# ywq/psnerf

Measured on AMD Instinct MI355X. Metric: ray-samples/sec (train step) on BEAR stage2, higher is better.
Workload: dtype f32

## Files before the change

include/psnerf_hip.h:

```cpp
#ifndef PSNERF_HIP_H
#define PSNERF_HIP_H

#include <stdint.h>

#ifdef __cplusplus
extern "C" {
#endif

#define PSN_OK 0
#define PSN_E_ARG (-1)
#define PSN_E_LAUNCH (-2)
#define PSN_E_UNSUPPORTED (-3)

const char* psn_last_error(void);
int psn_version(void);

int psn_composite_fwd(const float* alpha, const float* rgb, int64_t n_rays, int n_samples, int white_bg,
                      float* weights, float* rgb_out, float* acc_out, void* stream);
int psn_composite_bwd(const float* alpha, const float* rgb, const float* d_rgb_out, const float* d_acc_out,
                      int64_t n_rays, int n_samples, int white_bg, float* d_alpha, float* d_rgb, void* stream);

int psn_pe_encode(const float* x, int64_t n, int n_freqs, float scale, float* out, int out_stride, void* stream);
int psn_app_input(const float* p, const float* v, const float* normal, int64_t n, int n_freqs, float* out, void* stream);

// ... 135 lines not shown
    int n_layers;
    int n_out;
    int out_act;
    int in_kt_a;
    int in_kt_b;
    int init_stride;
    int w_format;
    PsnMlpLayer layers[PSN_MLP_MAX_LAYERS];
} PsnMlpDesc;

int psn_mlp_pack_layer(const float* W, int64_t ldw, int rows, int cols, int transpose, int n_mt, int k_tiles, float* dst,
                       void* stream);

#define PSN_PACK_MAX_ITEMS 24
typedef struct {
    const float* W;
    float* dst;
    int64_t ldw;
    int rows, cols, transpose, n_mt, k_tiles;
    int format;
} PsnPackItem;
int psn_mlp_pack_layers(int n_items, const PsnPackItem* items, void* stream);

typedef struct {
    const float* tab_a; int64_t a_div, a_mod; const float* tab_b; int64_t b_div, b_mod; const float* init_a; const float* init_b;
    float* const* save_ptrs; unsigned long long* const* save_bits_ptrs; int64_t save_row0;
    const float* const* mask_ptrs; const float* const* aux2_ptrs; float* const* save2_ptrs;
    const float* act_init; int64_t act_init_rows; const float* rk_coef; const float* rk_basis; int rk_k; const uint32_t* dump_tiles;
    int64_t n_rows; float* out; const float* live_count; int64_t live_period;
} PsnMlpLaunch;
typedef struct { int chain, width16, src, trim, from_a, x3, tb_lds, pm_groups; int64_t blocks, pm_period; } PsnMlpPath;
int psn_mlp_launch(const PsnMlpDesc* desc, const float* packed_w, const float* packed_b, const PsnMlpLaunch* launch, PsnMlpPath* path,
                   void* stream);
int psn_mlp_last_path(PsnMlpPath* path);
int psn_mlp_block_order(int point_major);

#define PSN_SCATTER_MAX_ITEMS 16
typedef struct {
    const float* rows;
    float* dense;
    int64_t row_stride, col_stride;
    int B, C;
    float fill;
} PsnScatterItem;
int psn_scatter_rows(int n_items, const PsnScatterItem* items, const int* inv, int64_t N, int64_t Ns, void* stream);
int psn_gather_rows(int n_items, const PsnScatterItem* items, const int64_t* idx, int64_t N, int64_t Ns, void* stream);
int psn_gather_rows_valid(int n_items, const PsnScatterItem* items, const int64_t* idx, const int* inv, int64_t N, int64_t Ns, void* stream);

int psn_secant_step(const float* occ, float tau, float* d_pred, float* d_low, float* d_high, float* f_low, float* f_high,
                    const float* origin, const float* dir, float* p_mid, int64_t n, void* stream);

int psn_first_crossing(const float* occ, const float* far, const float* u, const float* omu, float near, float tau,
// ... 272 lines not shown
```

psnerf_amd/csrc/mlp_infer.hip:

```cpp
#include "common.h"
#include <stdlib.h>
#include <atomic>

namespace psn {

struct InferArgs {
    PsnMlpDesc d;
    const float* w;
    const float* b;
    const float* ta;
    int64_t a_div, a_mod;
    const float* tb;
    int64_t b_div, b_mod;
    const float* init_a;
    const float* init_b;
    int64_t n_rows;
    float* out;
    int n_bias;
    float* save[PSN_MLP_MAX_LAYERS];
    int64_t save_row0;
    const float* mask[PSN_MLP_MAX_LAYERS];
    const float* aux2[PSN_MLP_MAX_LAYERS];
    float* save2[PSN_MLP_MAX_LAYERS];
    const float* act_init;
// ... 2 lines not shown
    const float* rk_coef;
    const float* rk_basis;
    int rk_k;
    const long long* n_rows_dev;
    const int64_t* out_rows;
    const float* ray_o;
    const float* ray_d;
    const float* bracket;
    float tau, pe_scale;
    int n_iter, pe_octaves;
    const float* far;
    const float* u;
    const float* omu;
    float near;
    int n_steps;
    int* skip;
    unsigned long long* n_blocks;
    const float* live_count;
    int64_t live_period;
    unsigned long long* save_bits[PSN_MLP_MAX_LAYERS];
    int tb_lds;
    int64_t pm_period;
    int pm_groups;
};

constexpr int kStageFloats = 8192;
constexpr int kWaves = 4;

template <int NMT, int NACC, bool ASMDMA, typename RequestNext>
__device__ __forceinline__ void stage_compute(floatx4 (&acc)[NACC], const floatx4& b0, const floatx4& b1,
                                              const float4* __restrict__ wl, int lane, RequestNext request_next) {
    if constexpr (NMT >= 8) {
        constexpr int GE = NMT / 8;
        constexpr int NG = 2 * GE;
        float4 a[2][8];
#pragma unroll
        for (int m = 0; m < 8; ++m) a[0][m] = wl[m * 64 + lane];
        __builtin_amdgcn_sched_barrier(0);
        constexpr int NPW = NMT / 2;
        if constexpr (ASMDMA) {
#pragma unroll
            for (int g = 0; g < NG; ++g) {
                const int e = g / GE, m0 = (g % GE) * 8;
                const floatx4& bs = e ? b1 : b0;
                const float4(&ag)[8] = a[g & 1];
#pragma unroll
// ... 171 lines not shown
    } else {
    const unsigned voff = lane * 16;
    switch (j & 3) {
        case 0: lds_dma_16<0>(base, lds, voff); break;
        case 1: lds_dma_16<1024>(base, lds, voff); break;
        case 2: lds_dma_16<2048>(base, lds, voff); break;
        default: lds_dma_16<3072>(base, lds, voff); break;
    }
    }
}
template <int NBLK, bool ASMDMA>
__device__ __forceinline__ void stage_load(const float* __restrict__ gsrc, float* lds_dst, int wave, int lane) {
#pragma unroll
    for (int j = 0; j < NBLK / kWaves; ++j) stage_piece<NBLK, ASMDMA>(gsrc, lds_dst, wave, lane, j);
}

__device__ __forceinline__ floatx4 ld4(const float* p) {
    float4 t = *reinterpret_cast<const float4*>(p);
    floatx4 v;
    v[0] = t.x; v[1] = t.y; v[2] = t.z; v[3] = t.w;
    return v;
}
__device__ __forceinline__ void st4(float* p, const floatx4& v) { *reinterpret_cast<float4*>(p) = make_float4(v[0], v[1], v[2], v[3]); }

template <int CODE, int NMT, bool FROMA = false>
__device__ __forceinline__ void chain_activation(floatx4 (&acc)[NMT], floatx4 (&act)[NMT], const float* __restrict__ p1,
                                                 const float* __restrict__ p2, float* __restrict__ d1, float* __restrict__ d2,
                                                 const uint32_t m1, const uint32_t m2, const unsigned long long sign_bits = 0) {
    constexpr bool kFromA = FROMA && (CODE == PSN_ACT_MUL_AUX || CODE == PSN_ACT_MUL2 || CODE == PSN_ACT_SOFTPLUS_BWD);
    constexpr bool kNeed1 = CODE == PSN_ACT_RELU_MASK || CODE == PSN_ACT_MUL_AUX || CODE == PSN_ACT_MUL2 || CODE == PSN_ACT_SOFTPLUS_BWD;
    constexpr bool kNeed2 = CODE == PSN_ACT_MUL2 || CODE == PSN_ACT_SOFTPLUS_BWD;
    constexpr bool kSecond = CODE == PSN_ACT_SOFTPLUS100 || CODE == PSN_ACT_MUL2 || CODE == PSN_ACT_MUL_AUX;
    floatx4 t1[NMT], t2[NMT];
    if constexpr (kNeed1) {
#pragma unroll
        for (int mt = 0; mt < NMT; ++mt) t1[mt] = ld4(p1 + mt * 16);
    }
    if constexpr (kNeed2) {
#pragma unroll
        for (int mt = 0; mt < NMT; ++mt) t2[mt] = ld4(p2 + mt * 16);
    }
    if constexpr (CODE == PSN_ACT_HEAD) {
        if (d1 != nullptr) {
#pragma unroll
            for (int mt = 0; mt < NMT; ++mt)
                if ((m1 >> mt) & 1) st4(d1 + mt * 16, acc[mt]);
// ... 205 lines not shown
    for (int i = tid; i < g.n_bias; i += kWaves * 64) bias_lds[i] = g.b[i];
    const float* tb_lds = nullptr;
    if constexpr (!CHAIN && SRC == 0) {
        if (g.init_b != nullptr && g.tb_lds != 0 && g.n_bias + g.d.init_stride <= PSN_MLP_MAX_LAYERS * 256) {
            const int64_t r_first = blk_ * (kWaves * 16), r_last_ = r_first + kWaves * 16 - 1;
            const int64_t r_last = r_last_ < n_rows_eff ? r_last_ : n_rows_eff - 1;
            if (r_first / g.b_div == r_last / g.b_div) {
                const int64_t ib0 = (r_first / g.b_div) % g.b_mod;
                float* dst = bias_lds + PSN_MLP_MAX_LAYERS * 256 - g.d.init_stride;
                const float* src = g.init_b + ib0 * (int64_t)g.d.init_stride;
                for (int i = tid; i < g.d.init_stride; i += kWaves * 64) dst[i] = src[i];
                tb_lds = dst;
            }
        }
    }

    floatx4 act[NMT];
    floatx4 acc[NMT];
#pragma unroll
    for (int mt = 0; mt < NMT; ++mt)
#pragma unroll
        for (int r = 0; r < 4; ++r) act[mt][r] = 0.f;
    if constexpr (CHAIN) {
        if (g.act_init != nullptr) {
            const bool has_row = rowc < g.act_init_rows;
            const float* ap = g.act_init + (has_row ? rowc : 0) * W + 4 * lg;
#pragma unroll
            for (int mt = 0; mt < NMT; ++mt) {
                float4 t = *reinterpret_cast<const float4*>(ap + mt * 16);
                act[mt][0] = has_row ? t.x : 0.f; act[mt][1] = has_row ? t.y : 0.f; act[mt][2] = has_row ? t.z : 0.f; act[mt][3] = has_row ? t.w : 0.f;
            }
#pragma unroll
            for (int mt = 0; mt < NMT; ++mt) asm volatile("" : "+v"(act[mt]));
        }
    }

    int gstage = 0;
    int pending_dump = 0;
    int pending_stages = 0;
    const bool dump_row = row < n_rows_eff && row >= g.save_row0;
    const bool wave_dumps = __builtin_amdgcn_ballot_w64(dump_row) != 0;

#define PSN_STAGE(NMT, B0, B1, S_IDX)                                                                       \
    {                                                                                                       \
         \
        wait_for_weights<NMT>(pending_stages > 0 ? pending_dump : 0);                                       \
// ... 69 lines not shown
                    }
                }
                if (tb_lds != nullptr) {
#pragma unroll
                    for (int mt = 0; mt < NMT; ++mt) {
                        const float4 u = *reinterpret_cast<const float4*>(tb_lds + L.init_off + mt * 16 + 4 * lg);
                        acc[mt][0] += u.x;
                        acc[mt][1] += u.y;
                        acc[mt][2] += u.z;
                        acc[mt][3] += u.w;
                    }
                } else if (init_b_row != nullptr) {
#pragma unroll
                    for (int mt = 0; mt < NMT; ++mt) {
                        float4 u = *reinterpret_cast<const float4*>(init_b_row + L.init_off + mt * 16 + 4 * lg);
                        acc[mt][0] += u.x;
                        acc[mt][1] += u.y;
                        acc[mt][2] += u.z;
                        acc[mt][3] += u.w;
                    }
                }
                if constexpr (CHAIN) {
                    if (g.rk_coef != nullptr) {
                        for (int c = 0; c < g.rk_k; ++c) {
                            const float cf = g.rk_coef[rowc * g.rk_k + c];
                            const float* bp2 = g.rk_basis + (int64_t)c * g.d.init_stride + L.init_off + 4 * lg;
#pragma unroll
                            for (int mt = 0; mt < NMT; ++mt) {
                                const float4 u = *reinterpret_cast<const float4*>(bp2 + mt * 16);
                                acc[mt][0] = fmaf(cf, u.x, acc[mt][0]);
                                acc[mt][1] = fmaf(cf, u.y, acc[mt][1]);
                                acc[mt][2] = fmaf(cf, u.z, acc[mt][2]);
                                acc[mt][3] = fmaf(cf, u.w, acc[mt][3]);
                            }
                        }
                    }
                }
            }
        }
        if (L.n_kt_act > 0) {
#pragma unroll
            for (int kt = 0; kt < NMT / 2 - 1; ++kt) PSN_STAGE(NMT, act[2 * kt], act[2 * kt + 1], kt)
            if (!TRIM || L.n_kt_act == NMT / 2) PSN_STAGE(NMT, act[NMT - 2], act[NMT - 1], NMT / 2 - 1)
        }
        if constexpr (SRC != 0) {
            if (L.n_kt_in > 0) {
                if constexpr (SRC == 2 || SRC == 3) {
                    PSN_STAGE(NMT, xq[0], xq[1], L.n_kt_act)
                    PSN_STAGE(NMT, xq[2], xq[3], L.n_kt_act + 1)
                } else {
#pragma unroll
                    for (int kt = 0; kt < 2; ++kt) {
                        const floatx4 x0 = compute_xin_tile(2 * kt), x1 = compute_xin_tile(2 * kt + 1);
                        PSN_STAGE(NMT, x0, x1, L.n_kt_act + kt)
                    }
                }
            }
        } else if (L.n_kt_in > 0) {
// ... 490 lines not shown
static psn::InferArgs base_args(const PsnMlpDesc& d, const float* packed_w, const float* packed_b, int64_t n_rows, float* out) {
    psn::InferArgs a = {};
    a.d = d; a.w = packed_w; a.b = packed_b; a.a_div = 1; a.a_mod = 1; a.b_div = 1; a.b_mod = 1; a.n_rows = n_rows; a.out = out;
    const int width = d.layers[0].n_mt * 32;
    a.n_bias = d.n_out > 0 ? (d.n_layers - 1) * width + (d.n_out > 32 ? 64 : 32) : d.n_layers * width;
    for (int l = 0; l < PSN_MLP_MAX_LAYERS; ++l) { a.save_tiles[l] = 0xFFFFFFFFu; a.save2_tiles[l] = 0xFFFFFFFFu; }
    return a;
}

static int mlp_infer_plan(const PsnMlpDesc* desc, const float* packed_w, const float* packed_b, const PsnMlpLaunch& o, psn::InferArgs& a,
                          PsnMlpPath& p) {
    using namespace psn;
    p = {};
    PSN_CHECK_ARG(desc && packed_w && packed_b && (o.out || desc->n_out == 0), "mlp_infer: null pointer");
    const PsnMlpDesc& d = *desc;
    PSN_CHECK_ARG(d.n_layers >= 1 && d.n_layers <= PSN_MLP_MAX_LAYERS, "mlp_infer: n_layers=%d", d.n_layers);
    PSN_CHECK_ARG(d.in_kt_a >= 0 && d.in_kt_b >= 0 && d.in_kt_a + d.in_kt_b <= 4, "mlp_infer: input tiles %d+%d", d.in_kt_a, d.in_kt_b);
    bool uses_in = false, uses_init = false;
    for (int l = 0; l < d.n_layers; ++l) {
        uses_in = uses_in || d.layers[l].n_kt_in > 0;
        uses_init = uses_init || d.layers[l].init_off >= 0;
    }
    PSN_CHECK_ARG(!uses_in || (o.tab_a && d.in_kt_a >= 1 && (d.in_kt_b == 0 || o.tab_b)), "mlp_infer: input table missing");
    PSN_CHECK_ARG((o.rk_coef == nullptr) == (o.rk_basis == nullptr) && (o.rk_coef == nullptr ? o.rk_k == 0 : (o.rk_k >= 1 && o.rk_k <= 4)),
                  "mlp_infer: rank-k init needs coefficients, basis and 1 <= k <= 4 (k=%d)", o.rk_k);
    PSN_CHECK_ARG(!uses_init || ((o.init_a || o.rk_coef) && d.init_stride >= 64 && d.init_stride % 4 == 0), "mlp_infer: init table missing");
    PSN_CHECK_ARG((((uintptr_t)o.rk_basis) & 15) == 0, "mlp_infer: rk_basis must be 16-byte aligned");
    PSN_CHECK_ARG((((uintptr_t)o.init_a | (uintptr_t)o.init_b) & 15) == 0, "mlp_infer: init tables must be 16-byte aligned");
    PSN_CHECK_ARG(d.n_out >= 0 && d.n_out <= 64, "mlp_infer: n_out=%d", d.n_out);
    PSN_CHECK_ARG(o.a_div >= 1 && o.a_mod >= 1 && (d.in_kt_b == 0 || (o.b_div >= 1 && o.b_mod >= 1)), "mlp_infer: bad index map");
    PSN_CHECK_ARG((((uintptr_t)o.tab_a | (uintptr_t)o.tab_b | (uintptr_t)packed_w | (uintptr_t)packed_b) & 15) == 0,
                  "mlp_infer: buffers must be 16-byte aligned");
    PSN_CHECK_ARG(o.save_bits_ptrs == nullptr || o.save_ptrs != nullptr, "mlp_infer: save_bits_ptrs needs save_ptrs (the sign bits are those of the dumps)");
    PSN_CHECK_ARG((o.live_count != nullptr) == (o.live_period != 0), "mlp_infer: live_count and live_period go together (live_count %s, period=%lld)",
                  o.live_count ? "given" : "is null", (long long)o.live_period);
    PSN_CHECK_ARG(d.n_out == 0 || d.n_layers >= 2, "mlp_infer: a final layer needs at least one hidden layer in front of it (n_layers=%d)", d.n_layers);
    const int hid = d.layers[0].n_mt;
    PSN_CHECK_ARG(hid == 8 || hid == 4 || hid == 2, "mlp_infer: hidden layers must be 256, 128 or 64 wide (n_mt = 8, 4, 2), got n_mt=%d", hid);
    const int width = hid * 32;
    for (int l = 0; l < d.n_layers; ++l) {
        const PsnMlpLayer& L = d.layers[l];
        const bool last = d.n_out > 0 && l == d.n_layers - 1;
        PSN_CHECK_ARG(L.n_mt == (last ? (d.n_out > 32 ? 2 : 1) : hid), "mlp_infer: layer %d n_mt=%d (hidden layers share one width; final: 1, or 2 for 33..64 outputs)", l, L.n_mt);
        PSN_CHECK_ARG(L.n_kt_in >= 0 && L.n_kt_in <= d.in_kt_a + d.in_kt_b, "mlp_infer: layer %d n_kt_in=%d", l, L.n_kt_in);
        PSN_CHECK_ARG(!last || (L.n_kt_in == 0 && L.n_kt_act == hid), "mlp_infer: the final layer reads the hidden activations only");
        PSN_CHECK_ARG(L.b_off == (int64_t)l * width, "mlp_infer: biases must be packed back to back (one hidden width per layer)");
        PSN_CHECK_ARG(L.n_kt_act == 0 || L.n_kt_act == hid || (L.n_kt_act == hid - 1 && hid > 1), "mlp_infer: layer %d n_kt_act=%d (0, n_mt - 1 or n_mt)", l, L.n_kt_act);
        PSN_CHECK_ARG(l > 0 || L.n_kt_act == 0 || o.act_init != nullptr, "mlp_infer: layer 0 cannot read activations without act_init");
        PSN_CHECK_ARG(L.n_kt_in + L.n_kt_act >= 1 || (l == 0 && L.init_off >= 0 && d.n_layers > 1), "mlp_infer: layer %d has no input", l);
        PSN_CHECK_ARG(L.init_off < 0 || (!last && L.init_off + width <= d.init_stride && L.init_off % 4 == 0), "mlp_infer: layer %d bad init_off", l);
// ... 13 lines not shown
        a.aux2[l] = (o.aux2_ptrs != nullptr && in_range) ? o.aux2_ptrs[l] : nullptr;
        a.save2[l] = (o.save2_ptrs != nullptr && in_range) ? o.save2_ptrs[l] : nullptr;
        PSN_CHECK_ARG(((((uintptr_t)a.mask[l]) | ((uintptr_t)a.aux2[l]) | ((uintptr_t)a.save2[l])) & 15) == 0,
                      "mlp_infer: aux / dump tensors must be 16-byte aligned");
        if (in_range) {
            const int act = d.layers[l].act;
            const bool need1 = act == PSN_ACT_RELU_MASK || act == PSN_ACT_MUL_AUX || act == PSN_ACT_MUL2 || act == PSN_ACT_SOFTPLUS_BWD || act == PSN_ACT_RELU_BITS ||
                               act == PSN_ACT_MUL_AUX_A || act == PSN_ACT_MUL2_A || act == PSN_ACT_SOFTPLUS_BWD_A;
            const bool need2 = act == PSN_ACT_MUL2 || act == PSN_ACT_SOFTPLUS_BWD || act == PSN_ACT_MUL2_A || act == PSN_ACT_SOFTPLUS_BWD_A;
            PSN_CHECK_ARG(act >= PSN_ACT_NONE && act <= PSN_ACT_SOFTPLUS_BWD_A, "mlp_infer: layer %d unknown activation %d", l, act);
            PSN_CHECK_ARG(!need1 || a.mask[l] != nullptr, "mlp_infer: layer %d needs aux operand 1", l);
            PSN_CHECK_ARG(!need2 || a.aux2[l] != nullptr, "mlp_infer: layer %d needs aux operand 2", l);
            PSN_CHECK_ARG(act != PSN_ACT_HEAD || a.save[l] != nullptr, "mlp_infer: a HEAD layer needs a dump tensor");
            const bool second = act == PSN_ACT_SOFTPLUS100 || act == PSN_ACT_MUL_AUX || act == PSN_ACT_MUL2 || act == PSN_ACT_MUL_AUX_A || act == PSN_ACT_MUL2_A;
            PSN_CHECK_ARG(a.save2[l] == nullptr || second, "mlp_infer: layer %d (activation %d) has no second value to dump", l, act);
        }
    }
    for (int l = 0; l < PSN_MLP_MAX_LAYERS; ++l) PSN_CHECK_ARG((((uintptr_t)a.save[l]) & 15) == 0, "mlp_infer: save buffers must be 16-byte aligned");
    const int rows_per_block = kWaves * 16;
    int64_t blocks = (o.n_rows + rows_per_block - 1) / rows_per_block;
    a.act_init = o.act_init;
    a.act_init_rows = o.act_init_rows;
    a.rk_coef = o.rk_coef; a.rk_basis = o.rk_basis; a.rk_k = o.rk_k;
    for (int l = 0; o.dump_tiles != nullptr && l < PSN_MLP_MAX_LAYERS; ++l) {
        a.save_tiles[l] = o.dump_tiles[l];
        a.save2_tiles[l] = o.dump_tiles[PSN_MLP_MAX_LAYERS + l];
    }
    PSN_CHECK_ARG((((uintptr_t)o.act_init) & 15) == 0, "mlp_infer: act_init must be 16-byte aligned");
    PSN_CHECK_ARG(o.act_init == nullptr || (o.act_init_rows >= 1 && o.act_init_rows <= o.n_rows), "mlp_infer: act_init_rows=%lld of %lld rows", (long long)o.act_init_rows, (long long)o.n_rows);
    bool chain = o.act_init != nullptr || o.rk_coef != nullptr || o.dump_tiles != nullptr;
    for (int l = 0; l < d.n_layers; ++l)
        chain = chain || d.layers[l].act > PSN_ACT_SOFTPLUS100 || a.save2[l] != nullptr || a.mask[l] != nullptr || a.aux2[l] != nullptr;
    PSN_CHECK_ARG(d.n_out <= 32 || (chain && hid == 8), "mlp_infer: 33..64 outputs are built for the 256-wide chain engine only (n_out=%d)", d.n_out);
    for (int l = 0; l < PSN_MLP_MAX_LAYERS; ++l) {
        a.save_bits[l] = (o.save_bits_ptrs != nullptr && l < n_hidden) ? o.save_bits_ptrs[l] : nullptr;
        PSN_CHECK_ARG(a.save_bits[l] == nullptr || (!chain && a.save[l] != nullptr && (((uintptr_t)a.save_bits[l]) & 7) == 0),
                      "mlp_infer: sign-bit words (layer %d) go with an activation dump of a plain forward launch", l);
    }
    PSN_CHECK_ARG(o.live_count == nullptr || (!chain && d.n_out >= 1 && o.live_period >= 64 && o.live_period % 64 == 0 && o.save_row0 >= 0 &&
                                              o.save_row0 % o.live_period == 0 && o.save_row0 <= o.n_rows),
                  "mlp_infer_padded: needs the lean variant, outputs, a period that is a multiple of 64 and save_row0 a multiple of the period (period=%lld save_row0=%lld)",
                  (long long)o.live_period, (long long)o.save_row0);
    a.live_count = o.live_count; a.live_period = o.live_period > 0 ? o.live_period : 1;
    static const int tb = [] { const char* e = getenv("PSN_TB_LDS"); return (e != nullptr && e[0] == '0') ? 0 : 1; }();
    a.tb_lds = tb;
    const bool pair = !chain && o.a_div == 1 && (o.tab_b != nullptr || o.init_b != nullptr) && o.b_div == o.a_mod && o.b_div >= rows_per_block &&
// ... 119 lines not shown
```

psnerf_amd/hip.py:

```python
import ctypes
import os

import torch

from . import cabi

_HERE = os.path.dirname(os.path.abspath(__file__))
LIB_PATH = os.path.join(_HERE, 'libpsnerf_hip.so')

if not os.path.exists(LIB_PATH):
    raise ImportError(
        'psnerf_amd: %s is missing. Build it with `python -m psnerf_amd.build` (hipcc, gfx950). '
        'There is no fallback path.' % LIB_PATH)
_lib = ctypes.CDLL(LIB_PATH)

HEADER_PATH = os.path.join(_HERE, '..', 'include', 'psnerf_hip.h')
if not os.path.exists(HEADER_PATH):
    raise ImportError('psnerf_amd: %s is missing: the binding is derived from it. There is no fallback path.' % HEADER_PATH)

_constants, _structs, SIGNATURES = cabi.parse(HEADER_PATH)
globals().update({_k[len('PSN_'):]: _v for _k, _v in _constants.items()})
globals().update(_structs)
MAX_LAYERS = MLP_MAX_LAYERS
for _name, (_res, _args) in SIGNATURES.items():
# ... 950 lines not shown
            rows, cols = (W.shape[1], W.shape[0]) if transpose else (W.shape[0], W.shape[1])
            e.W, e.dst, e.ldw = W.data_ptr(), dst.data_ptr(), W.stride(0)
            e.rows, e.cols, e.transpose, e.n_mt, e.k_tiles = rows, cols, int(transpose), n_mt, k_tiles
        _check(_lib.psn_mlp_pack_layers(len(chunk), ctypes.addressof(arr), _stream()), 'mlp_pack_layers')


class block_order(object):

    def __init__(self, order):
        assert order in ('point', 'row'), order
        self.order = order

    def __enter__(self):
        self.saved = _lib.psn_mlp_block_order(1 if self.order == 'point' else 0)
        return self

    def __exit__(self, *exc):
        _lib.psn_mlp_block_order(self.saved)
        return False


def mlp_infer(desc, packed_w, packed_b, tab_a, a_div, a_mod, tab_b, b_div, b_mod, n_rows, out=None, init_a=None,
              init_b=None, save=None, save_row0=0, mask=None, aux2=None, save2=None, act_init=None, macs_per_row=None,
              rank_init=None, save_tiles=None, save2_tiles=None, act_init_rows=None, live=None, save_bits=None, path=None):
    o, keep = PsnMlpLaunch(), []
    if save_tiles is not None or save2_tiles is not None:
        tiles_arr = (ctypes.c_uint32 * (2 * MAX_LAYERS))(*([0xFFFFFFFF] * (2 * MAX_LAYERS)))
        for base, lst in ((0, save_tiles), (MAX_LAYERS, save2_tiles)):
            for l, m in enumerate(lst or []):
                if m is not None:
                    tiles_arr[base + l] = int(m)
        keep.append(tiles_arr)
        o.dump_tiles = ctypes.addressof(tiles_arr)
    if rank_init is not None:
        rk_coef, rk_basis = rank_init
        o.rk_k = rk_k = rk_basis.shape[0]
        assert rk_coef.shape == (n_rows, rk_k) and rk_coef.is_contiguous() and rk_basis.is_contiguous() and 1 <= rk_k <= 4
        assert rk_basis.shape[1] == desc.init_stride, 'rank_init: the basis rows are init_stride floats'
        o.rk_coef, o.rk_basis = _tptr(rk_coef, 'rk_coef'), _tptr(rk_basis, 'rk_basis')
    if act_init is not None:
        o.act_init_rows = n_rows if act_init_rows is None else act_init_rows
        assert act_init.is_contiguous() and act_init.shape[0] >= o.act_init_rows, 'act_init: fewer rows than act_init_rows'
        o.act_init = _tptr(act_init, 'act_init')
    if out is None and desc.n_out > 0:
        out = torch.empty(n_rows, desc.n_out, device=packed_w.device, dtype=torch.float32)
    n_hidden = desc.n_layers - 1 if desc.n_out > 0 else desc.n_layers

    def ptr_array(lst, n, name, words=None):
        if lst is None:
            return None
        assert len(lst) == n, '%s: expected %d entries' % (name, n)
        is_words = lambda t: t.dtype == torch.int64 if words is None else words
        keep.append((ctypes.c_void_p * n)(*[None if t is None else (_bits_ptr(t, name) if is_words(t) else _tptr(t, name)) for t in lst]))
        return ctypes.addressof(keep[-1])

    o.mask_ptrs, o.aux2_ptrs, o.save2_ptrs = (ptr_array(lst, desc.n_layers, name) for lst, name in ((mask, 'mask'), (aux2, 'aux2'), (save2, 'save2')))
    o.save_ptrs, o.save_bits_ptrs = ptr_array(save, n_hidden, 'save', False), ptr_array(save_bits, n_hidden, 'save_bits', True)
    for t, b in zip(save or [], save_bits or []):
        assert b is None or (t is not None and b.shape == (t.shape[0], 4))
    if live is not None:
        cnt, period = live
        assert cnt.is_cuda and cnt.dtype == torch.float32 and cnt.numel() == 1 and int(period) >= 1
# ... 617 lines not shown
```

psnerf_amd/ops.py:

```python
import collections

import torch

from . import fused, hip


HITS = collections.Counter()


def _hit(name):
    HITS[name] += 1


import os as _os0
STRICT = _os0.environ.get('PSN_STRICT', '0') == '1'
FALLBACKS = collections.Counter()


def fallback(name, tensor=None, why=''):
    if tensor is not None and not getattr(tensor, 'is_cuda', False):
        return
    FALLBACKS[name] += 1
    if STRICT:
        raise RuntimeError('psnerf_amd.ops.STRICT: %s left the fused engines on a device tensor%s' % (name, (' (' + why + ')') if why else ''))
# ... 185 lines not shown
        ctx.skip_at = skip_at
        return out

    @staticmethod
    def backward(ctx, d_out):
        tab_a, tab_b, in_cols = ctx.saved_tensors[:3]
        params = [p.detach().requires_grad_(True) for p in ctx.saved_tensors[3:]]
        nA, nB = tab_a.shape[0], tab_b.shape[0]
        ta = tab_a.detach().requires_grad_(ctx.needs_input_grad[0])
        tb = tab_b.detach().requires_grad_(ctx.needs_input_grad[1])
        with torch.enable_grad():
            x = torch.cat([ta.tile(nB, 1), tb.repeat_interleave(nA, dim=0)], dim=1)
            out = ReluMLP.apply(x, in_cols, ctx.skip_at, False, *params)
            wanted = [t for t in [ta, tb] + params if t.requires_grad]
            got = torch.autograd.grad(out, wanted, d_out, allow_unused=True)
        it = iter(got)
        res = []
        for t in [ta, tb]:
            res.append(next(it) if t.requires_grad else None)
        pg = [next(it) for _ in params]
        return (res[0], res[1], None, None) + tuple(pg)


class SplitRows(torch.autograd.Function):

    @staticmethod
    def forward(ctx, t, k):
        ctx.k, ctx.shape = k, t.shape
        return t[:k], t[k:]

    @staticmethod
    def backward(ctx, ga, gb):
        k, shape = ctx.k, ctx.shape
        if ga is None:
            ga = gb.new_zeros((k,) + tuple(shape[1:]))
        if gb is None:
            gb = ga.new_zeros((shape[0] - k,) + tuple(shape[1:]))
        return torch.cat([ga, gb], dim=0), None


class ScatterRows(torch.autograd.Function):

    @staticmethod
    def forward(ctx, idx, inv, specs, *rows):
        _hit('ScatterRows')
        ctx.set_materialize_grads(False)
        ctx.specs, ctx.n_pix, ctx.ns = specs, inv.numel(), idx.numel()
        ctx.save_for_backward(idx, inv)
        return tuple(hip.scatter_rows(list(specs), [r.detach() for r in rows], inv, inv.numel(), idx.numel()))

    @staticmethod
    def backward(ctx, *grads):
        idx, inv = ctx.saved_tensors
        sel = [k for k, g in enumerate(grads) if g is not None and ctx.needs_input_grad[3 + k]]
        out = [None] * len(grads)
        if sel:
            got = hip.gather_rows([ctx.specs[k] for k in sel], [grads[k].contiguous() for k in sel], idx, ctx.n_pix, ctx.ns, inv=inv)
            for k, g in zip(sel, got):
                out[k] = g
        return (None, None, None) + tuple(out)

# ... 532 lines not shown
    def backward(ctx, g):
        n, d_x, chains = ctx.meta
        sv = ctx.saved_tensors
        x, feat = sv[0], sv[1]
        H = sv[2:2 + n - 1]
        Ws = sv[2 + n - 1:]
        Q, dev = x.shape[0], x.device
        g = g.contiguous()
        DZ = [torch.empty(Q, 256, device=dev) for _ in range(n - 1)]
        d_feat = torch.empty(Q, 256, device=dev)
        d_normal = chains['bwd'](None, Q, a_div=1, a_mod=Q, rank_init=(g, Ws[n - 1].contiguous()),
                                 mask=[H[n - 2 - j] for j in range(n - 1)] + [None, None], save=DZ + [d_feat])
        dz0 = DZ[n - 2]
        items = [dict(A=dz0, B=x[:, :d_x], colsum=True), dict(A=dz0, B=feat)]
        items += [dict(A=DZ[n - 2 - l], B=H[l - 1], colsum=True) for l in range(1, n - 1)]
        res = hip.gemm_tn_grouped(items)
        grads = [torch.cat([res[0][0], res[1][0]], dim=1), res[0][1]]
        for l in range(1, n - 1):
            grads += [res[l + 1][0], res[l + 1][1]]
        grads += [hip.colsum(H[n - 2], row_weight=g), _rowsum_small(g)]
        return (None, d_normal, d_feat, None, None) + tuple(grads)


class FusedReluNet(torch.autograd.Function):

    @staticmethod
    def pack(Ws, bs, din, skip_at, final_sigmoid, width):
        with torch.no_grad():
            return fused.pack_relu_mlp(list(Ws), list(bs), din, 0, skip_at,
                                       out_act=hip.OUT_SIGMOID if final_sigmoid else hip.OUT_NONE, precompute=False, width=width)

    @staticmethod
    def forward(ctx, pe, din, skip_at, final_sigmoid, width, packed, *params):
        _hit('FusedReluNet')
        Ws, bs = params[0::2], params[1::2]
        n = len(Ws)
        Q = pe.shape[0]
        if packed is None:
            packed = FusedReluNet.pack(Ws, bs, din, skip_at, final_sigmoid, width)
        need = any(ctx.needs_input_grad[6:])
        H = [torch.empty(Q, width, device=pe.device) for _ in range(n - 1)] if need else None
        bits = _sign_bits(Q, n - 1, pe.device) if (need and RELU_SIGN_BITS) else None
        out = packed(pe, Q, save=H, save_bits=bits)
        if need:
            ctx.save_for_backward(pe, out, *H, *Ws)
            ctx.meta = (n, din, skip_at, final_sigmoid, width)
            ctx.bits = bits
        return out

    @staticmethod
    def backward(ctx, g):
        n, din, skip_at, final_sigmoid, width = ctx.meta
        sv = ctx.saved_tensors
        pe, out = sv[0], sv[1]
        H = sv[2:2 + n - 1]
        Ws = sv[2 + n - 1:]
        Q, dev = pe.shape[0], pe.device
        g = g.contiguous()
        if final_sigmoid:
            g = torch.ops.aten.sigmoid_backward(g, out)
        bits = ctx.bits
        chain = fused.pack_relu_bwd(list(Ws), skip_at, width=width, bits=bits is not None, x3=CHAIN_X3)
        DZ = [torch.empty(Q, width, device=dev) for _ in range(n - 1)]
        masks = [(bits if bits is not None else H)[n - 2 - j] for j in range(n - 1)]
        if Ws[n - 1].shape[0] <= 4:
            chain(None, Q, a_div=1, a_mod=Q, rank_init=(g, Ws[n - 1].contiguous()), mask=masks, save=DZ)
        else:
            dh = hip.gemm(g, Ws[n - 1].contiguous())
            chain(None, Q, a_div=1, a_mod=Q, init_a_direct=dh, mask=masks, save=DZ)
        x_in = pe[:, :din]
        items = [dict(A=g, B=H[n - 2], colsum=True)]
        where = [(n - 1, 'w')]
        for l in range(n - 2, -1, -1):
            dz = DZ[n - 2 - l]
            if l == 0:
                items.append(dict(A=dz, B=x_in, colsum=True))
                where.append((0, 'w'))
            else:
                items.append(dict(A=dz, B=H[l - 1], colsum=True))
                where.append((l, 'w'))
                if l - 1 == skip_at:
                    items.append(dict(A=dz, B=x_in))
                    where.append((l, 'x'))
        res = hip.gemm_tn_grouped(items)
        dW, dWx, db = [None] * n, [None] * n, [None] * n
        for (l, kind), (C, cs) in zip(where, res):
            if kind == 'w':
                dW[l], db[l] = C, cs
            else:
                dWx[l] = C
# ... 143 lines not shown
```

psnerf_amd/stage2/renderer.py:

```python
import contextlib
import os

import numpy as np
import torch
import torch.nn as nn
import torch.nn.functional as F

from .. import fused, hip, ops

PE_STRIDE = 64


def camera_rays(uv, pose, intrinsics):
    fx, fy = intrinsics[:, 0, 0], intrinsics[:, 1, 1]
    cx, cy = intrinsics[:, 0, 2], intrinsics[:, 1, 2]
    z = torch.ones_like(uv[:, :, 0])
    x = (uv[:, :, 0] - cx.unsqueeze(-1)) / fx.unsqueeze(-1) * z
    y = (uv[:, :, 1] - cy.unsqueeze(-1)) / fy.unsqueeze(-1) * z
    R = pose[:, :3, :3]
    d = x.unsqueeze(-1) * R[:, None, :, 0] + y.unsqueeze(-1) * R[:, None, :, 1] + z.unsqueeze(-1) * R[:, None, :, 2]
    return F.normalize(d, dim=2), pose[:, :3, 3]


class MLP(fused.PackCached, nn.Module):
# ... 317 lines not shown
        if ns > 0:
            normal = gather(normals) if not self.normal_mlp else normal_s
            with on_side():
                if (uv.is_cuda and uv.shape[0] == 1 and uv.dtype == torch.float32 and tuple(pose.shape[1:]) == (4, 4)
                        and tuple(intr.shape[1:]) == (4, 4)):
                    pts2c = hip.camera_rays(uv.contiguous(), pose.contiguous().float(), intr.contiguous().float(), idx, scale=-1.0)
                else:
                    ray_dirs, _ = camera_rays(uv, pose, intr)
                    pts2c = -gather(ray_dirs)
            light_dir = input['light_direction']
            cols = self._cols(self.n_freqs, device)
            if pe_x is None:
                pe_x = self._memo('pe_x', input, lambda: self._pe(surf, self.n_freqs))
            pe_j = None
            with on_side():
              if self.xyz_jitter_std > 0:
                nz = noise.get('xyz')
                if nz is None:
                    nz = torch.empty_like(surf).normal_(0.0, self.xyz_jitter_std)
                def brdf_both():
                    pe_both = torch.cat([pe_x, self._pe(surf + nz, self.n_freqs)], dim=0)
                    return self.albedo_net(pe_both, cols), self.rough_net(pe_both, cols)
                albedo_both, rough_both = self._memo('brdf_both', input, brdf_both)
                albedo, albedo_j = ops.SplitRows.apply(albedo_both, ns)
                if sg:
                    rough_both = F.relu(rough_both)
                rough, rough_j = ops.SplitRows.apply(rough_both, ns)
              else:
                albedo, rough = self._memo('brdf', input, lambda: (self.albedo_net(pe_x, cols), self.rough_net(pe_x, cols)))
              if albedo_new is not None:
                albedo = torch.from_numpy(albedo_new).to(device)[None].expand_as(albedo)
              if sg:
                weights = rough if self.xyz_jitter_std > 0 else F.relu(rough)
                if basis_new is not None:
                    wn = torch.zeros_like(weights)
                    if self.specular_rgb:
                        wn.view(-1, 3, self.nbasis // 3)[:, :, basis_new] = 2 ** basis_new / 100
                    else:
                        wn.view(-1, 1, self.nbasis)[:, :, basis_new] = 2 ** basis_new / 100
                    weights = wn.reshape(-1, self.nbasis)
                weight_values = scatter(weight_values, weights)
            if side is not None:
                main = torch.cuda.current_stream(device)
                main.wait_stream(side)
                for t_ in (pts2c, normal_s, albedo_both if self.xyz_jitter_std > 0 else albedo, rough_both if self.xyz_jitter_std > 0 else rough,
                           weights if sg else None, out_n.get('normal_jitter').rows if 'normal_jitter' in out_n else None):
                    if torch.is_tensor(t_):
                        t_.record_stream(main)
            light_int = input.get('light_intensity', self.light_int)
            vis = None
# ... 93 lines not shown
```

Baseline: 113.1 million.

## Fuse split-concat, relu gate and sigmoid backward into rank-k MLP backward init

Gradients from SplitRows and the ReLU gate are now carried lazily as a (lo, hi, split, gate) record instead of being concatenated and thresholded. The fused MLP backward kernel takes both coefficient sources plus an optional gate/sigmoid program, builds the effective coefficients in LDS per wave, and can write them out. Rank-k init is widened from at most 4 to up to 32, and the backward weight packing moves into forward. This removes cat, threshold_backward, sigmoid_backward and a separate GEMM launch, at the cost of extra kernel branching, an LDS stash, and autograd-tensor attribute tricks.

```diff
diff --git a/include/psnerf_hip.h b/include/psnerf_hip.h
--- a/include/psnerf_hip.h
+++ b/include/psnerf_hip.h
@@ -181,12 +181,15 @@
 } PsnPackItem;
 int psn_mlp_pack_layers(int n_items, const PsnPackItem* items, void* stream);
 
+#define PSN_MLP_MAX_RANK 32
+enum { PSN_RK_SPLIT = 1, PSN_RK_GATE = 2, PSN_RK_SIGMOID = 4 };
 typedef struct {
     const float* tab_a; int64_t a_div, a_mod; const float* tab_b; int64_t b_div, b_mod; const float* init_a; const float* init_b;
     float* const* save_ptrs; unsigned long long* const* save_bits_ptrs; int64_t save_row0;
     const float* const* mask_ptrs; const float* const* aux2_ptrs; float* const* save2_ptrs;
     const float* act_init; int64_t act_init_rows; const float* rk_coef; const float* rk_basis; int rk_k; const uint32_t* dump_tiles;
     int64_t n_rows; float* out; const float* live_count; int64_t live_period;
+    int rk_prog; int64_t rk_split; const float* rk_coef2; const float* rk_y; float* rk_out;
 } PsnMlpLaunch;
 typedef struct { int chain, width16, src, trim, from_a, x3, tb_lds, pm_groups; int64_t blocks, pm_period; } PsnMlpPath;
 int psn_mlp_launch(const PsnMlpDesc* desc, const float* packed_w, const float* packed_b, const PsnMlpLaunch* launch, PsnMlpPath* path,
diff --git a/psnerf_amd/csrc/mlp_infer.hip b/psnerf_amd/csrc/mlp_infer.hip
--- a/psnerf_amd/csrc/mlp_infer.hip
+++ b/psnerf_amd/csrc/mlp_infer.hip
@@ -48,6 +48,13 @@
     int tb_lds;
     int64_t pm_period;
     int pm_groups;
+    struct Rk {
+        int prog;
+        int64_t split;
+        const float* coef2;
+        const float* y;
+        float* out;
+    } rk;
 };
 
 constexpr int kStageFloats = 8192;
@@ -265,6 +272,56 @@
     return v;
 }
 __device__ __forceinline__ void st4(float* p, const floatx4& v) { *reinterpret_cast<float4*>(p) = make_float4(v[0], v[1], v[2], v[3]); }
+
+constexpr int kRkStash = 16 * PSN_MLP_MAX_RANK;
+struct __attribute__((packed, aligned(4))) RkPiece { float v[4]; };
+__device__ __forceinline__ void rk_effective(const InferArgs& g, const int64_t row0, const int lane, float* stash) {
+    const int k = g.rk_k;
+    const InferArgs::Rk& rk = g.rk;
+    for (int p = lane; p < 4 * k; p += 64) {
+        floatx4 v = {0.f, 0.f, 0.f, 0.f};
+        const int64_t e0 = row0 * k + 4 * p, n_el = g.n_rows * k;
+        const int64_t s_el = (rk.prog & PSN_RK_SPLIT) ? rk.split * k : n_el;
+        const bool use_y = (rk.prog & (PSN_RK_GATE | PSN_RK_SIGMOID)) != 0;
+        const bool whole = e0 + 4 <= n_el;
+        floatx4 y = {0.f, 0.f, 0.f, 0.f};
+        if (whole && (e0 + 4 <= s_el || e0 >= s_el)) {
+            if (e0 >= s_el) {
+                const RkPiece t = *reinterpret_cast<const RkPiece*>(rk.coef2 + (e0 - s_el));
+                v[0] = t.v[0]; v[1] = t.v[1]; v[2] = t.v[2]; v[3] = t.v[3];
+            } else {
+                v = ld4(g.rk_coef + e0);
+            }
+            if (use_y) y = ld4(rk.y + e0);
+        } else {
+#pragma unroll
+            for (int j = 0; j < 4; ++j) {
+                const int64_t e = e0 + j;
+                if (e < n_el) {
+                    v[j] = e >= s_el ? rk.coef2[e - s_el] : g.rk_coef[e];
+                    if (use_y) y[j] = rk.y[e];
+                }
+            }
+        }
+        if (rk.prog & PSN_RK_GATE) {
+#pragma unroll
+            for (int j = 0; j < 4; ++j) v[j] = y[j] <= 0.0f ? 0.0f : v[j];
+        }
+        if (rk.prog & PSN_RK_SIGMOID) {
+#pragma unroll
+            for (int j = 0; j < 4; ++j) v[j] = v[j] * (1.0f - y[j]) * y[j];
+        }
+        if (rk.out != nullptr) {
+            if (whole) st4(rk.out + e0, v);
+            else {
+#pragma unroll
+                for (int j = 0; j < 4; ++j)
+                    if (e0 + j < n_el) rk.out[e0 + j] = v[j];
+            }
+        }
+        st4(stash + 4 * p, v);
+    }
+}
 
 template <int CODE, int NMT, bool FROMA = false>
 __device__ __forceinline__ void chain_activation(floatx4 (&acc)[NMT], floatx4 (&act)[NMT], const float* __restrict__ p1,
@@ -516,6 +573,7 @@
 #pragma unroll
         for (int r = 0; r < 4; ++r) act[mt][r] = 0.f;
     if constexpr (CHAIN) {
+        if (g.rk_coef != nullptr) rk_effective(g, blk_ * (kWaves * 16) + wave * 16, lane, smem + kStageFloats + wave * kRkStash);
         if (g.act_init != nullptr) {
             const bool has_row = rowc < g.act_init_rows;
             const float* ap = g.act_init + (has_row ? rowc : 0) * W + 4 * lg;
@@ -631,8 +689,9 @@
                 }
                 if constexpr (CHAIN) {
                     if (g.rk_coef != nullptr) {
+                        const float* cfp = smem + kStageFloats + wave * kRkStash + lj * g.rk_k;
                         for (int c = 0; c < g.rk_k; ++c) {
-                            const float cf = g.rk_coef[rowc * g.rk_k + c];
+                            const float cf = cfp[c];
                             const float* bp2 = g.rk_basis + (int64_t)c * g.d.init_stride + L.init_off + 4 * lg;
 #pragma unroll
                             for (int mt = 0; mt < NMT; ++mt) {
@@ -643,6 +702,7 @@
                                 acc[mt][3] = fmaf(cf, u.w, acc[mt][3]);
                             }
                         }
+                        asm volatile("s_waitcnt lgkmcnt(0)" ::: "memory");
                     }
                 }
             }
@@ -1179,10 +1239,23 @@
         uses_init = uses_init || d.layers[l].init_off >= 0;
     }
     PSN_CHECK_ARG(!uses_in || (o.tab_a && d.in_kt_a >= 1 && (d.in_kt_b == 0 || o.tab_b)), "mlp_infer: input table missing");
-    PSN_CHECK_ARG((o.rk_coef == nullptr) == (o.rk_basis == nullptr) && (o.rk_coef == nullptr ? o.rk_k == 0 : (o.rk_k >= 1 && o.rk_k <= 4)),
-                  "mlp_infer: rank-k init needs coefficients, basis and 1 <= k <= 4 (k=%d)", o.rk_k);
+    PSN_CHECK_ARG((o.rk_coef == nullptr) == (o.rk_basis == nullptr) && (o.rk_coef == nullptr ? o.rk_k == 0 : (o.rk_k >= 1 && o.rk_k <= PSN_MLP_MAX_RANK)),
+                  "mlp_infer: rank-k init needs coefficients, basis and 1 <= k <= %d (k=%d)", PSN_MLP_MAX_RANK, o.rk_k);
     PSN_CHECK_ARG(!uses_init || ((o.init_a || o.rk_coef) && d.init_stride >= 64 && d.init_stride % 4 == 0), "mlp_infer: init table missing");
     PSN_CHECK_ARG((((uintptr_t)o.rk_basis) & 15) == 0, "mlp_infer: rk_basis must be 16-byte aligned");
+    PSN_CHECK_ARG((((uintptr_t)o.rk_coef | (uintptr_t)o.rk_y | (uintptr_t)o.rk_out) & 15) == 0 && (((uintptr_t)o.rk_coef2) & 3) == 0,
+                  "mlp_infer: rk_coef, rk_y and rk_out must be 16-byte aligned (rk_coef2: 4-byte)");
+    for (int l = 1; l < d.n_layers; ++l)
+        PSN_CHECK_ARG(o.rk_coef == nullptr || d.layers[l].init_off < 0, "mlp_infer: a rank-k init starts layer 0 only (layer %d has init_off >= 0)", l);
+    PSN_CHECK_ARG((o.rk_prog & ~(PSN_RK_SPLIT | PSN_RK_GATE | PSN_RK_SIGMOID)) == 0, "mlp_infer: unknown rk_prog bits 0x%x", o.rk_prog);
+    PSN_CHECK_ARG(o.rk_coef != nullptr || (o.rk_prog == 0 && o.rk_coef2 == nullptr && o.rk_y == nullptr && o.rk_out == nullptr && o.rk_split == 0),
+                  "mlp_infer: the output-side program (rk_prog, rk_coef2, rk_y, rk_out, rk_split) belongs to a rank-k init");
+    PSN_CHECK_ARG((o.rk_coef2 != nullptr) == ((o.rk_prog & PSN_RK_SPLIT) != 0), "mlp_infer: a second coefficient source and PSN_RK_SPLIT go together (rk_coef2 %s, rk_prog=0x%x)",
+                  o.rk_coef2 ? "given" : "is null", o.rk_prog);
+    PSN_CHECK_ARG((o.rk_prog & PSN_RK_SPLIT) ? (o.rk_split >= 0 && o.rk_split <= o.n_rows) : o.rk_split == 0, "mlp_infer: rk_split=%lld of %lld rows",
+                  (long long)o.rk_split, (long long)o.n_rows);
+    PSN_CHECK_ARG((o.rk_y != nullptr) == ((o.rk_prog & (PSN_RK_GATE | PSN_RK_SIGMOID)) != 0), "mlp_infer: the forward output rk_y goes with PSN_RK_GATE / PSN_RK_SIGMOID (rk_y %s, rk_prog=0x%x)",
+                  o.rk_y ? "given" : "is null", o.rk_prog);
     PSN_CHECK_ARG((((uintptr_t)o.init_a | (uintptr_t)o.init_b) & 15) == 0, "mlp_infer: init tables must be 16-byte aligned");
     PSN_CHECK_ARG(d.n_out >= 0 && d.n_out <= 64, "mlp_infer: n_out=%d", d.n_out);
     PSN_CHECK_ARG(o.a_div >= 1 && o.a_mod >= 1 && (d.in_kt_b == 0 || (o.b_div >= 1 && o.b_mod >= 1)), "mlp_infer: bad index map");
@@ -1242,6 +1315,7 @@
     a.act_init = o.act_init;
     a.act_init_rows = o.act_init_rows;
     a.rk_coef = o.rk_coef; a.rk_basis = o.rk_basis; a.rk_k = o.rk_k;
+    a.rk.prog = o.rk_prog; a.rk.split = o.rk_split; a.rk.coef2 = o.rk_coef2; a.rk.y = o.rk_y; a.rk.out = o.rk_out;
     for (int l = 0; o.dump_tiles != nullptr && l < PSN_MLP_MAX_LAYERS; ++l) {
         a.save_tiles[l] = o.dump_tiles[l];
         a.save2_tiles[l] = o.dump_tiles[PSN_MLP_MAX_LAYERS + l];
diff --git a/psnerf_amd/hip.py b/psnerf_amd/hip.py
--- a/psnerf_amd/hip.py
+++ b/psnerf_amd/hip.py
@@ -996,7 +996,8 @@
 
 def mlp_infer(desc, packed_w, packed_b, tab_a, a_div, a_mod, tab_b, b_div, b_mod, n_rows, out=None, init_a=None,
               init_b=None, save=None, save_row0=0, mask=None, aux2=None, save2=None, act_init=None, macs_per_row=None,
-              rank_init=None, save_tiles=None, save2_tiles=None, act_init_rows=None, live=None, save_bits=None, path=None):
+              rank_init=None, save_tiles=None, save2_tiles=None, act_init_rows=None, live=None, save_bits=None, path=None,
+              rank_prog=None):
     o, keep = PsnMlpLaunch(), []
     if save_tiles is not None or save2_tiles is not None:
         tiles_arr = (ctypes.c_uint32 * (2 * MAX_LAYERS))(*([0xFFFFFFFF] * (2 * MAX_LAYERS)))
@@ -1009,9 +1010,31 @@
     if rank_init is not None:
         rk_coef, rk_basis = rank_init
         o.rk_k = rk_k = rk_basis.shape[0]
-        assert rk_coef.shape == (n_rows, rk_k) and rk_coef.is_contiguous() and rk_basis.is_contiguous() and 1 <= rk_k <= 4
+        rp = rank_prog or {}
+        split = rp.get('split')
+        rows1 = n_rows if split is None else int(split[0])
+        assert rk_coef.shape == (rows1, rk_k) and rk_coef.is_contiguous() and rk_basis.is_contiguous() and 1 <= rk_k <= MLP_MAX_RANK
+        if rows1 == 0:
+            rk_coef = split[1]
         assert rk_basis.shape[1] == desc.init_stride, 'rank_init: the basis rows are init_stride floats'
+        if rk_coef.data_ptr() % 16:
+            rk_coef = rk_coef.clone()
+        keep.append(rk_coef)
         o.rk_coef, o.rk_basis = _tptr(rk_coef, 'rk_coef'), _tptr(rk_basis, 'rk_basis')
+        if split is not None:
+            assert split[1].shape == (n_rows - rows1, rk_k), 'rank_prog: the second source holds the rows behind the split'
+            o.rk_prog, o.rk_split, o.rk_coef2 = o.rk_prog | RK_SPLIT, rows1, _tptr(split[1] if rows1 < n_rows else rk_coef, 'rk_coef2')
+        if rp.get('gate'):
+            o.rk_prog |= RK_GATE
+        if rp.get('sigmoid'):
+            o.rk_prog |= RK_SIGMOID
+        for key, field in (('y', 'rk_y'), ('out', 'rk_out')):
+            t = rp.get(key)
+            if t is not None:
+                assert t.shape == (n_rows, rk_k), 'rank_prog: %s is [n_rows, k]' % key
+                setattr(o, field, _tptr(t, field))
+    else:
+        assert rank_prog is None, 'rank_prog belongs to a rank_init'
     if act_init is not None:
         o.act_init_rows = n_rows if act_init_rows is None else act_init_rows
         assert act_init.is_contiguous() and act_init.shape[0] >= o.act_init_rows, 'act_init: fewer rows than act_init_rows'
diff --git a/psnerf_amd/ops.py b/psnerf_amd/ops.py
--- a/psnerf_amd/ops.py
+++ b/psnerf_amd/ops.py
@@ -231,21 +231,66 @@
         return (res[0], res[1], None, None) + tuple(pg)
 
 
+LAZY_ROWS = True
+RowsGrad = collections.namedtuple('RowsGrad', 'lo hi split gate')
+
+
+def _lazy_producer(t):
+    return LAZY_ROWS and t.is_cuda and t.dtype == torch.float32 and t.dim() == 2 and type(t.grad_fn).__name__ in ('FusedReluNetBackward', 'GateReluBackward')
+
+
+def _rows_grad(g):
+    return getattr(g, '_psn_rows', None)
+
+
+def _carry(like, shape, rows):
+    c = like.new_empty(shape)
+    c._psn_rows = rows
+    return c
+
+
 class SplitRows(torch.autograd.Function):
 
     @staticmethod
-    def forward(ctx, t, k):
+    def forward(ctx, t, k, lazy=False):
         ctx.k, ctx.shape = k, t.shape
+        ctx.lazy = bool(lazy) and _lazy_producer(t) and 0 < k < t.shape[0]
         return t[:k], t[k:]
 
     @staticmethod
     def backward(ctx, ga, gb):
         k, shape = ctx.k, ctx.shape
+        if ctx.lazy and ga is not None and gb is not None and _rows_grad(ga) is None and _rows_grad(gb) is None:
+            return _carry(ga, shape, RowsGrad(ga.contiguous(), gb.contiguous(), k, None)), None, None
         if ga is None:
             ga = gb.new_zeros((k,) + tuple(shape[1:]))
         if gb is None:
             gb = ga.new_zeros((shape[0] - k,) + tuple(shape[1:]))
-        return torch.cat([ga, gb], dim=0), None
+        return torch.cat([ga, gb], dim=0), None, None
+
+
+class GateRelu(torch.autograd.Function):
+
+    @staticmethod
+    def forward(ctx, x, lazy=False):
+        y = torch.relu(x)
+        ctx.lazy = bool(lazy) and _lazy_producer(x)
+        ctx.save_for_backward(y)
+        return y
+
+    @staticmethod
+    def backward(ctx, g):
+        y, = ctx.saved_tensors
+        rows = _rows_grad(g)
+        if rows is not None:
+            if ctx.lazy and rows.gate is None:
+                return _carry(g, g.shape, rows._replace(gate=y)), None
+            g = torch.cat([rows.lo, rows.hi], dim=0)
+        return torch.ops.aten.threshold_backward(g, y, 0), None
+
+
+def gate_relu(x, lazy=False):
+    return GateRelu.apply(x, lazy)
 
 
 class ScatterRows(torch.autograd.Function):
@@ -824,6 +869,9 @@
         return (None, d_normal, d_feat, None, None) + tuple(grads)
 
 
+PACK_BWD_IN_FORWARD = True
+
+
 class FusedReluNet(torch.autograd.Function):
 
     @staticmethod
@@ -848,6 +896,7 @@
             ctx.save_for_backward(pe, out, *H, *Ws)
             ctx.meta = (n, din, skip_at, final_sigmoid, width)
             ctx.bits = bits
+            ctx.chain = fused.pack_relu_bwd(list(Ws), skip_at, width=width, bits=bits is not None, x3=CHAIN_X3) if PACK_BWD_IN_FORWARD else None
         return out
 
     @staticmethod
@@ -858,16 +907,30 @@
         H = sv[2:2 + n - 1]
         Ws = sv[2 + n - 1:]
         Q, dev = pe.shape[0], pe.device
-        g = g.contiguous()
-        if final_sigmoid:
-            g = torch.ops.aten.sigmoid_backward(g, out)
         bits = ctx.bits
-        chain = fused.pack_relu_bwd(list(Ws), skip_at, width=width, bits=bits is not None, x3=CHAIN_X3)
+        chain = ctx.chain if ctx.chain is not None else fused.pack_relu_bwd(list(Ws), skip_at, width=width, bits=bits is not None, x3=CHAIN_X3)
         DZ = [torch.empty(Q, width, device=dev) for _ in range(n - 1)]
         masks = [(bits if bits is not None else H)[n - 2 - j] for j in range(n - 1)]
-        if Ws[n - 1].shape[0] <= 4:
-            chain(None, Q, a_div=1, a_mod=Q, rank_init=(g, Ws[n - 1].contiguous()), mask=masks, save=DZ)
+        rows = _rows_grad(g)
+        if rows is not None and Ws[n - 1].shape[0] > hip.MLP_MAX_RANK:
+            g = torch.cat([rows.lo, rows.hi], dim=0)
+            if rows.gate is not None:
+                g = torch.ops.aten.threshold_backward(g, rows.gate, 0)
+            rows = None
+        if Ws[n - 1].shape[0] <= hip.MLP_MAX_RANK:
+            prog = None
+            if rows is not None or final_sigmoid:
+                g_in = rows.lo if rows is not None else g.contiguous()
+                g = torch.empty(Q, Ws[n - 1].shape[0], device=dev)
+                prog = dict(split=(rows.split, rows.hi) if rows is not None else None, gate=rows is not None and rows.gate is not None,
+                            sigmoid=final_sigmoid, y=out if (final_sigmoid or (rows is not None and rows.gate is not None)) else None, out=g)
+            else:
+                g_in = g = g.contiguous()
+            chain(None, Q, a_div=1, a_mod=Q, rank_init=(g_in, Ws[n - 1].contiguous()), rank_prog=prog, mask=masks, save=DZ)
         else:
+            g = g.contiguous()
+            if final_sigmoid:
+                g = torch.ops.aten.sigmoid_backward(g, out)
             dh = hip.gemm(g, Ws[n - 1].contiguous())
             chain(None, Q, a_div=1, a_mod=Q, init_a_direct=dh, mask=masks, save=DZ)
         x_in = pe[:, :din]
diff --git a/psnerf_amd/stage2/renderer.py b/psnerf_amd/stage2/renderer.py
--- a/psnerf_amd/stage2/renderer.py
+++ b/psnerf_amd/stage2/renderer.py
@@ -363,10 +363,10 @@
                     pe_both = torch.cat([pe_x, self._pe(surf + nz, self.n_freqs)], dim=0)
                     return self.albedo_net(pe_both, cols), self.rough_net(pe_both, cols)
                 albedo_both, rough_both = self._memo('brdf_both', input, brdf_both)
-                albedo, albedo_j = ops.SplitRows.apply(albedo_both, ns)
+                albedo, albedo_j = ops.SplitRows.apply(albedo_both, ns, True)
                 if sg:
-                    rough_both = F.relu(rough_both)
-                rough, rough_j = ops.SplitRows.apply(rough_both, ns)
+                    rough_both = ops.gate_relu(rough_both, True)
+                rough, rough_j = ops.SplitRows.apply(rough_both, ns, True)
               else:
                 albedo, rough = self._memo('brdf', input, lambda: (self.albedo_net(pe_x, cols), self.rough_net(pe_x, cols)))
               if albedo_new is not None:
```

Result: no change. 113.6 million (median of 6 runs) (+0.4%).
